# zhouzypaul/fql

Measured on AMD Instinct MI355X. Metric: FQL gradient-steps/s (batch=256), higher is better.
Workload: dtype f32

## Files before the change

### experiments/ab_inproc.py

```python
import os
import statistics
import sys
import time

sys.path.insert(0, os.path.dirname(os.path.dirname(os.path.abspath(__file__))))
import fql_amd
from tests.util import make_problem

envs = [dict(kv.split('=', 1) for kv in a.split()) if a.strip() and a.strip() != '-' else {} for a in sys.argv[1:3]]
rounds = int(sys.argv[3]) if len(sys.argv) > 3 else 7
n = int(sys.argv[4]) if len(sys.argv) > 4 else 300
prec = sys.argv[5] if len(sys.argv) > 5 else 'fp32'
B = int(sys.argv[6]) if len(sys.argv) > 6 else 256
H = 512
cfg, ds, batch, noise = make_problem(29, 8, B, (H,) * 4, seed=3)
cfg['precision'] = prec
agents = []
from fql_amd import _cabi
for e in envs:
    lib = e.pop('LIB', None)
    if lib:
        _cabi.LIB_PATH = os.path.abspath(lib)
        _cabi._lib = None
    e_show = dict(e, **({'LIB': lib} if lib else {}))
# ... 2 lines not shown
    a = fql_amd.FQLAgent.create(0, batch['observations'][:1], batch['actions'][:1], cfg)
    a.upload_dataset(ds)
    for _ in range(30):
        a.update_from_dataset(B)
    a.synchronize()
    agents.append(a)
    for k in e:
        del os.environ[k]
    e.update(e_show)
res = [[], []]
for r in range(rounds):
    for i, a in enumerate(agents):
        for _ in range(10):
            a.update_from_dataset(B)
        a.synchronize()
        t0 = time.perf_counter()
        for _ in range(n):
            a.update_from_dataset(B)
        a.synchronize()
        res[i].append((time.perf_counter() - t0) / n * 1e6)
for i, e in enumerate(envs):
    print(f'{"AB"[i]} {e}: median {statistics.median(res[i]):.1f} us/update  (min {min(res[i]):.1f}, max {max(res[i]):.1f})  = {1e6 / statistics.median(res[i]):.0f} updates/s')
print(f'B / A time: {statistics.median(res[1]) / statistics.median(res[0]):.4f}')
```

### fql_amd/csrc/fql_engine.hip

```cpp
#include "../../include/fql_amd.h"
#include "fql_kernels.h"
#include "fql_conv.h"
#include "fql_chain.h"
#include "fql_aux.h"
#include "fql_ifql.h"
#include "fql_rebrac.h"
#include "fql_sac.h"
#include "fql_bc.h"
#include "fql_iql.h"
#include "fql_iqld.h"
#include "fql_cfgrl.h"
#include <hip/hip_ext.h>
#include "fql_aql.h"

#include <algorithm>
#include <cmath>
#include <cstdarg>
#include <cstdio>
#include <cstdlib>
#include <cstring>
#include <map>
#include <memory>
#include <random>
#include <string>
// ... 138 lines not shown
    PrepArgs prep;
    PostOsArgs postos;
    LossCriticArgs lc;
    LossQArgs lq;
    LossBcArgs lb;
    LossActorArgs la;
    EulerFinishArgs ef;
    ConvArgs conv;
    PoolArgs pool;
    PoolBwdArgs poolb;
    ConvWgradArgs cw;
    ConvWredArgs cwr;
    EncDzArgs edz;
    ChainArgs chain;
    const ConvWprepTask* wprep_tasks = nullptr;
    int wprep_n = 0;
    int cw_grid = 0;
    int adam_c0 = 0, adam_n = -1;
    int adam_c1 = 0, adam_n1 = 0;
    int adam_polyak = -1;
    float adam_lr = 0.f;
    DevState* adam_st = nullptr;
    int fin_mode = 0;
    Bound k;
    int level = 0;
    int lane = 0;
    std::vector<int> deps;
};

struct Launch {
    OpType type;
    int grid = 0, ntasks = 0;
    size_t lds = 0;
    void* table = nullptr;
    Op op;
    bool pool_fused = false;
    int lane = 0;
    bool tmt2 = false, kbig = false, euler = false;
    double macs = 0.0;
    void *table_w = nullptr, *table_l = nullptr, *table_m = nullptr;
    int n_w = 0, n_l = 0, tile_w = 0, tile_l = 0, tile_m = 0;
    std::vector<GemmTask> dg_tasks;
    std::vector<GemmTask> h_gemm;
    std::vector<WgradTask> h_wgrad;
    std::vector<LnBwdTask> h_ln;
    std::vector<int> waits;
// ... 249 lines not shown
    float* in_noise[5] = {nullptr, nullptr, nullptr, nullptr, nullptr};
    int64_t* in_idx = nullptr;
    float *X_os = nullptr, *X_bc = nullptr, *X_eu = nullptr, *X_c1 = nullptr, *X_c2 = nullptr, *X_ct = nullptr;
    float *vel = nullptr, *w_rew = nullptr, *w_mask = nullptr, *w_act = nullptr, *tgt = nullptr;
    float *X_e0 = nullptr, *C0 = nullptr, *Abuf[2] = {nullptr, nullptr}, *Vpart = nullptr;
    bool fused_euler = false;
    bool use_chain = false;
    int fill_lane_full = 1;
    std::vector<float*> wf_bc;
    float *wf_w0 = nullptr, *wf_w4 = nullptr;
    WfragTask* d_wfrag = nullptr;
    int wfrag_n = 0, wfrag_grid = 0;
    std::vector<void*> chain_allocs;
    bool split_build = false;
    bool wide_tiles = false;
    bool split_ok = false;
    int vp_tiles = 0;
    int num_cus = 0;
    PassBuf p_os, p_os_bwd, p_bc, p_eu, p_c1[2], p_c2[2], p_ct[2];
    Program prog_fwdbwd, prog_opt, prog_loss;
    Program prog_opt_split;
    Program prog_full;
    int mod_chunk0[3] = {0, 0, 0}, mod_chunkn[3] = {0, 0, 0};
    Program prog_split;
    hipGraphExec_t split_exec[4] = {nullptr, nullptr, nullptr, nullptr};
    hipGraph_t split_graph[4] = {nullptr, nullptr, nullptr, nullptr};
    hipEvent_t ev_a = nullptr, ev_b = nullptr, ev_c = nullptr;
    bool split_begun = false;
    bool began = false;
    AqlRuntime aql;
    std::vector<AqlDispatch>* aql_rec = nullptr;
    bool last_update_aql = false;
    bool hip_dirty = true;
    void aql_drain() {
        if (!aql.up) return;
        try { aql.drain(); } catch (const AqlError& e) { throw HipError{e.msg}; }
    }

    float *ds_obs = nullptr, *ds_act = nullptr, *ds_rew = nullptr, *ds_mask = nullptr, *ds_nobs = nullptr;
    float* ds_row = nullptr;
    int64_t ds_size = 0, ds_cap = 0, ds_ptr = 0;
    unsigned char *ds_frames = nullptr, *ds_next_frames = nullptr;
    int64_t* ds_init = nullptr;
    int ds_fs = 0;
    float ds_paug = 0.f;
    float *rb_obs = nullptr, *rb_act = nullptr, *rb_rew = nullptr, *rb_mask = nullptr, *rb_nobs = nullptr;
// ... 397 lines not shown
        std::vector<int> range(n_train_leaves + 1, 0);
        for (const AdamChunk& c : ch) range[c.leaf + 1]++;
        for (int i = 0; i < n_train_leaves; ++i) range[i + 1] += range[i];
        {
            static const char* const trained[kNumKinds][3] = {
                {"modules_actor_bc_flow/", "modules_actor_onestep_flow/", "modules_critic/"},
                {"modules_actor_flow/", "modules_value/", "modules_critic/"},
                {"modules_actor/", "modules_critic/", "modules_critic/"},
                {"modules_actor/", "modules_alpha/", "modules_critic/"},
                {nullptr, nullptr, nullptr},
                {"modules_actor/", "modules_value/", "modules_critic/"},
                {"actor/", "value/", "critic/"},
                {nullptr, nullptr, nullptr}};
            const char* const* mods = trained[(int)kind];
            for (int m = 0; m < 3; ++m) {
                if (!mods[m]) { mod_chunk0[m] = 0; mod_chunkn[m] = n_chunks; continue; }
                int lo = 1 << 30, hi = -1;
                for (const Leaf& lf : leaves)
                    if (lf.trainable && lf.name.rfind(mods[m], 0) == 0) { lo = std::min(lo, lf.train_id); hi = std::max(hi, lf.train_id); }
                mod_chunk0[m] = range[lo];
                mod_chunkn[m] = range[hi + 1] - range[lo];
            }
        }
        HIP_CHECK(hipMalloc((void**)&d_leaf_range, range.size() * sizeof(int)));
        HIP_CHECK(hipMemcpy(d_leaf_range, range.data(), range.size() * sizeof(int), hipMemcpyHostToDevice));
        HIP_CHECK(hipMalloc((void**)&d_partials, (size_t)n_chunks * 4 * sizeof(float)));
        HIP_CHECK(hipMemset(d_partials, 0, (size_t)n_chunks * 4 * sizeof(float)));
    }

    const Leaf* find_leaf(const char* name) const {
        for (const Leaf& l : leaves)
            if (l.name == name) return &l;
        return nullptr;
    }
    static size_t leaf_count(const Leaf& l) {
        size_t n = 1;
        for (int i = 0; i < l.ndim; ++i) n *= (size_t)l.shape[i];
        return n;
    }
    void leaf_io(const Leaf& lf, float* arena, float* host, bool to_device) {
        HIP_CHECK(hipStreamSynchronize(stream));
        size_t ho = 0;
        for (const Segment& s : lf.segs) {
            HIP_CHECK(hipMemcpy2D(to_device ? (void*)(arena + s.off) : (void*)(host + ho), (to_device ? s.cols_p : s.cols) * sizeof(float),
                                  to_device ? (const void*)(host + ho) : (const void*)(arena + s.off),
                                  (to_device ? s.cols : s.cols_p) * sizeof(float), s.cols * sizeof(float), s.rows,
                                  to_device ? hipMemcpyHostToDevice : hipMemcpyDeviceToHost));
            ho += (size_t)s.rows * s.cols;
        }
    }
// ... 1168 lines not shown
                }
                else {
#define FQL_CHAIN_F32(HH, VV) FQL_LAUNCH((fql_chain_kernel<HH, VV>), dim3((L.op.chain.M / 16) * (HH / 32)), dim3(FQL_CHAIN_THREADS), FQL_CHAIN_LDS_BYTES(HH), s, ca)
                    if (cfg.actor_hidden[0] == 512) { if (ca.variant == 0) FQL_CHAIN_F32(512, 0); else if (ca.variant == 1) FQL_CHAIN_F32(512, 1); else if (ca.variant == 2) FQL_CHAIN_F32(512, 2); else FQL_CHAIN_F32(512, 3); }
                    else { if (ca.variant == 0) FQL_CHAIN_F32(256, 0); else if (ca.variant == 1) FQL_CHAIN_F32(256, 1); else if (ca.variant == 2) FQL_CHAIN_F32(256, 2); else FQL_CHAIN_F32(256, 3); }
#undef FQL_CHAIN_F32
                }
                break;
            }
            case OP_WFRAG:
                FQL_LAUNCH(fql_wfrag_kernel, dim3(wfrag_grid), dim3(FQL_THREADS), 0, s, (const WfragTask*)d_wfrag, wfrag_n, tl);
                break;
            case OP_DGRAD0: {
                Dgrad0Args a{};
                a.ntasks = (int)L.dg_tasks.size(); a.col0 = L.op.gemm.i1;
                for (int i = 0; i < a.ntasks; ++i) a.t[i] = L.dg_tasks[i];
                FQL_LAUNCH(fql_dgrad0_kernel, dim3(a.ntasks * (L.op.gemm.M / 16)), dim3(FQL_THREADS), 0, s, a);
                break;
            }
            case OP_HEAD_DGRAD:
                FQL_LAUNCH(fql_head_dgrad_kernel, dim3((L.op.gemm.M / 16) * (L.op.gemm.N / 64)), dim3(FQL_THREADS), 0, s, L.op.gemm);
                break;
            case OP_ADAM: {
                AdamArgs a{P, G, Mu, Nu, P + n_train, d_chunks, L.op.adam_st ? L.op.adam_st : d_state, d_partials, L.op.adam_c0,
                           L.op.adam_polyak >= 0 ? L.op.adam_polyak : (int)critic_size, L.op.adam_lr > 0.f ? L.op.adam_lr : cfg.lr, cfg.tau, tl,
                           L.op.adam_n1 > 0 ? L.op.adam_n : -1, L.op.adam_c1};
                FQL_LAUNCH(fql_adam_kernel, dim3(L.op.adam_n < 0 ? n_chunks : L.op.adam_n + L.op.adam_n1), dim3(FQL_THREADS), 0, s, a);
                break;
            }
            case OP_FINALIZE:
                FQL_LAUNCH(fql_finalize_kernel, dim3(1), dim3(FQL_THREADS), 0, s,
                                   FinalizeArgs{d_state, d_chunks, d_partials, d_leaf_range, n_chunks, n_train_leaves, L.op.fin_mode, tl});
                break;
            case OP_WGRAD: case OP_LNBWD: case OP_POSTOS: case OP_LOSS_CRITIC: case OP_LOSS_Q: case OP_LOSS_BC:
            case OP_PEC: case OP_XCHAIN: case OP_NUM_TYPES:
                throw HipError{"internal: op type " + std::to_string((int)L.type) + " has no launch of its own"};
            default: {
                const Bound& k = L.op.k;
                if (!k.fn) throw HipError{"internal: op type " + std::to_string((int)L.type) + " carries no bound launch"};
                alignas(16) unsigned char a[FQL_BOUND_BYTES];
                std::memcpy(a, k.args, (size_t)k.len);
                if (k.tl_at >= 0) std::memcpy(a + k.tl_at, &tl, sizeof tl);
                if (L.type == OP_IQLD_CFG) std::memcpy(a + offsetof(IqldCfgStepArgs, cfg), &sample_cfg, sizeof sample_cfg);
                void* argv[2] = {a + k.at[0], a + k.at[1]};
                if (aql_rec) aql_rec->push_back(AqlDispatch{k.fn, {k.grid, 1, 1}, {FQL_THREADS, 1, 1}, 0, std::vector<uint8_t>(a, a + k.len)});
                else if (prof_a) (void)hipExtLaunchKernel(k.fn, dim3(k.grid), dim3(FQL_THREADS), argv, 0, s, prof_a, prof_b, 0);
                else (void)hipLaunchKernel(k.fn, dim3(k.grid), dim3(FQL_THREADS), argv, 0, s);
                break;
            }
        }
    }

#undef FQL_LAUNCH
// ... 353 lines not shown
                if (t.K == 16 && t.N % 64 == 0 && t.M % 16 == 0 && (t.flags & GF_TRANS_B) && (t.flags & GF_GELUGRAD) && !(t.flags & (GF_BIAS | GF_RELUGRAD | GF_A_LN)) &&
                    cfg.precision != 1)
                    d.type = OP_HEAD_DGRAD;
                t.f0 = cfg.alpha * 2.0f / (float)(B * ad);
                d.reads.erase(std::remove(d.reads.begin(), d.reads.end(), (const void*)da), d.reads.end());
                for (const void* r : {(const void*)p_os.out, (const void*)tgt, (const void*)p_c2[0].dx0, (const void*)p_c2[1].dx0}) d.reads.push_back(r);
                d.writes.push_back(da);
                if (euler_finish_fused) {
                    const Net& nb = nets[NET_BC];
                    t.flags |= GF_A_EULFIN;
                    t.aux = Abuf[(fs - 1) & 1]; t.aux2 = Vpart; t.eb = P + nb.layers[nb.nl() - 1].b; t.f1 = 1.0f / (float)fs; t.ln_width = vp_tiles;
                    d.reads.erase(std::remove(d.reads.begin(), d.reads.end(), (const void*)tgt), d.reads.end());
                    for (const void* r : {(const void*)Abuf[(fs - 1) & 1], (const void*)Vpart, (const void*)(P + nb.layers[nb.nl() - 1].w)}) d.reads.push_back(r);
                    d.writes.push_back(tgt);
                }
            }
            if (euler_finish_fused) {
                const int keep = emit_lane;
                emit_lane = la_lane;
                push(pr, la_op);
                emit_lane = keep;
            }
            for (Op& w : os_w) {
                w.reads.push_back(p_os_bwd.dz[0]);
                emit_lane = 0;
                push(pr, w);
            }
            emit_lane = 0;
        }
        if (with_grads && visual) {
            place("enc", split_build ? 0 : 1, true);
            emit_encoder_backward(pr, eb_os, 0, B, p_os_bwd.dx0, nullptr, nets[NET_OS].in_p());
            if (enc_align) {
                emit_encoder_backward(pr, eb_c, 0, B, p_c1[0].dx0, p_c1[1].dx0, nets[NET_C0].in_p(), p_os_bwd.dx0);
                emit_encoder_backward(pr, eb_bc, 0, B, p_bc.dx0, nullptr, nets[NET_BC].in_p(), p_os_bwd.dx0);
            }
        }
        if (!with_grads) {
            Op op{};
            op.type = OP_FINALIZE;
            op.fin_mode = 0;
            op.reads = {I_CR, I_BC, I_Q, I_MSE, I_ACT};
            op.writes = {INFO};
            push(pr, op);
        }
    }

    void adam_for(Program& pr, int m, std::initializer_list<int> net_ids, int lane, int m2 = -1) {
        DevState* st = d_state;
            Op a{};
            a.type = OP_ADAM;
            a.adam_c0 = mod_chunk0[m]; a.adam_n = mod_chunkn[m];
            a.reads = {st};
            a.writes = {d_partials + mod_chunk0[m] * 4};
            if (m2 >= 0) { a.adam_c1 = mod_chunk0[m2]; a.adam_n1 = mod_chunkn[m2]; a.writes.push_back(d_partials + mod_chunk0[m2] * 4); }
            if (m2 == -2) {
                a.adam_c0 = 0; a.adam_n = -1;
                for (int mm = 0; mm < 3; ++mm) a.writes.push_back(d_partials + mod_chunk0[mm] * 4);
            }
            if (m == 2 && tgt) a.reads.push_back(tgt);
            for (int mm : {m, m2}) if (visual && mm >= 0) {
                const int m = mm;
                const int ei = m == 2 ? ENC_C : (m == 0 ? ENC_BC : ENC_OS);
                for (const EncStack& st : encs[ei].stacks)
                    for (const ConvL& c : st.conv) {
                        a.reads.push_back(G + c.w); a.reads.push_back(G + c.b);
                        a.writes.push_back(P + c.w);
                        if (m == 2) a.writes.push_back(P + n_train + c.w);
                    }
                const Layer& D = encs[ei].dense;
                a.reads.push_back(G + D.w); a.reads.push_back(G + D.b);
                a.writes.push_back(P + D.w);
                if (m == 2) a.writes.push_back(P + n_train + D.w);
            }
            for (int ni : net_ids)
                for (const Layer& L : nets[ni].layers) {
                    a.reads.push_back(G + L.w); a.reads.push_back(G + L.b);
                    a.writes.push_back(P + L.w);
                    if (L.ln) { a.reads.push_back(G + L.g); a.reads.push_back(G + L.be); a.writes.push_back(P + L.g); }
                    if (ni == NET_C0 || ni == NET_C1) a.writes.push_back(P + n_train + L.w);
                }
            emit_lane = lane;
            push(pr, a);
// ... 9 lines not shown
        } else {
            adam_for(pr, 2, {NET_C0, NET_C1, NET_BC, NET_OS}, 0, -2);
            if (use_chain) { emit_lane = 0; emit_wfrag(pr); }
        }
        Op f{};
        f.type = OP_FINALIZE;
        f.fin_mode = 1;
        f.reads = {d_partials + mod_chunk0[0] * 4, d_partials + mod_chunk0[1] * 4, d_partials + mod_chunk0[2] * 4, &st->info[0],
                   &st->info[4], &st->info[5], &st->info[7], &st->info[9]};
        f.writes = {&st->info[10], st};
        emit_lane = 0;
        push(pr, f);
    }
    void run_opt_split(hipStream_t s0, hipStream_t s1) {
        if (!ev_c) HIP_CHECK(hipEventCreateWithFlags(&ev_c, hipEventDisableTiming));
        if (!split_begun) HIP_CHECK(hipEventRecord(ev_c, s0));
        HIP_CHECK(hipStreamWaitEvent(s1, ev_c, 0));
        split_begun = false;
        const hipStream_t ls[FQL_LANES] = {s0, s1, s1, s1};
        run_launches(prog_opt_split, s0, ls, false);
    }

    void build_full_program(Program& pr) {
        build_step_program(pr, true);
        DevState* st = d_state;
        adam_for(pr, 2, {NET_C0, NET_C1, NET_BC}, fill_lane_full, 0);
        emit_wfrag(pr);
        adam_for(pr, 1, {NET_OS}, 0);
        Op f{};
        f.type = OP_FINALIZE;
        f.fin_mode = 1;
        f.reads = {d_partials + mod_chunk0[0] * 4, d_partials + mod_chunk0[1] * 4, d_partials + mod_chunk0[2] * 4, &st->info[0],
                   &st->info[4], &st->info[5], &st->info[7], &st->info[9]};
        f.writes = {&st->info[10], st};
        emit_lane = 0;
        push(pr, f);
    }

    FinalizeArgs fin_args(int do_grad_stats) const {
        return FinalizeArgs{d_state, d_chunks, d_partials, d_leaf_range, n_chunks, n_train_leaves, do_grad_stats, -1};
    }

    void build_ifql_program(Program& pr, bool with_grads) {
        const int od = cfg.obs_dim, ad = cfg.act_dim, ap = pad16(ad);
        DevState* st = d_state;
        const void *I_V = &st->info[IFQL_I_VALUE], *I_C = &st->info[IFQL_I_CRITIC], *I_A = &st->info[IFQL_I_ACTOR];
        wide_tiles = true;
        allow64 = true;
        emit_lane = 0;
        {
            Op op{};
            op.type = OP_IFQL_PREP;
            const IfqlPrepArgs iprep{d_src, st, seed, B, od, ad, nets[NET_OS].in_p(), nets[NET_C0].in_p(), nets[NET_BC].in_p(), ap,
                                     X_v, X_c1, X_bc, vel, w_rew, w_mask};
            op.k = bind(fql_ifql_prep_kernel, (iprep.B + 3) / 4, iprep);
            op.writes = {X_v, X_c1, X_bc, vel, w_rew, w_mask};
            push(pr, op);
        }
        emit_lane = 1;
// ... 1915 lines not shown
            std::vector<float> tab((size_t)(S + 1) * BC_EMB);
            for (int k = 0; k <= S; ++k) {
                const float t = (float)k / (float)S;
                const float ts = t * 10000.0f;
                for (int i = 0; i < BC_EMB / 2; ++i) {
                    const float freq = (float)std::exp(-std::log(10000.0) * (double)i / (double)(BC_EMB / 2));
                    const float arg = ts * freq;
                    tab[(size_t)k * BC_EMB + i] = (float)std::cos((double)arg);
                    tab[(size_t)k * BC_EMB + BC_EMB / 2 + i] = (float)std::sin((double)arg);
                }
            }
            HIP_CHECK(hipMalloc((void**)&h->d_emb, tab.size() * sizeof(float)));
            HIP_CHECK(hipMemcpy(h->d_emb, tab.data(), tab.size() * sizeof(float), hipMemcpyHostToDevice));
        }
        HIP_CHECK(hipMalloc((void**)&h->P, h->n_total * sizeof(float)));
        HIP_CHECK(hipMalloc((void**)&h->G, h->n_train * sizeof(float)));
        HIP_CHECK(hipMalloc((void**)&h->Mu, h->n_train * sizeof(float)));
        HIP_CHECK(hipMalloc((void**)&h->Nu, h->n_train * sizeof(float)));
        HIP_CHECK(hipMemset(h->G, 0, h->n_train * sizeof(float)));
        HIP_CHECK(hipMemset(h->Mu, 0, h->n_train * sizeof(float)));
        HIP_CHECK(hipMemset(h->Nu, 0, h->n_train * sizeof(float)));
        h->build_enc_weights();
        h->build_leaves();
        h->init_params();
        h->build_chain_weights();
        h->refresh_chain_weights(h->stream);
        HIP_CHECK(hipMalloc((void**)&h->d_state, sizeof(DevState)));
        if (h->own_info()) {
            HIP_CHECK(hipMalloc((void**)&h->iql_info, 2 * IQL_INFO_STRIDE * sizeof(float)));
            HIP_CHECK(hipMemset(h->iql_info, 0, 2 * IQL_INFO_STRIDE * sizeof(float)));
        }
        HIP_CHECK(hipMalloc((void**)&h->d_src, sizeof(SrcDesc)));
        HIP_CHECK(hipHostMalloc((void**)&h->h_src_ring, 64 * sizeof(SrcDesc), hipHostMallocDefault));
        HIP_CHECK(hipHostMalloc((void**)&h->h_info_ring, fql_engine::kInfoRing * 32 * sizeof(float), hipHostMallocDefault));
        for (auto& e : h->info_ev) HIP_CHECK(hipEventCreateWithFlags(&e, hipEventDisableTiming));
        DevState st{};
        st.rng_step = 0; st.adam_count = 0; st.train_step = 1; st.b1pow = 1.0; st.b2pow = 1.0; st.grad_scale = 1.0f; st.lam = 1.0f;
        const float ninf = -INFINITY, pinf = INFINITY;
        int bi; std::memcpy(&bi, &ninf, 4); st.gmax = bi >= 0 ? bi : bi ^ 0x7FFFFFFF;
        std::memcpy(&bi, &pinf, 4); st.gmin = bi >= 0 ? bi : bi ^ 0x7FFFFFFF;
        HIP_CHECK(hipMemcpy(h->d_state, &st, sizeof st, hipMemcpyHostToDevice));
        if (kind == AgentKind::IQLD) {
            HIP_CHECK(hipMalloc((void**)&h->d_state_a, sizeof(DevState)));
            HIP_CHECK(hipMemcpy(h->d_state_a, &st, sizeof st, hipMemcpyHostToDevice));
        }
        if (kind == AgentKind::CFGRL) {
// ... 2 lines not shown
            HIP_CHECK(hipHostMalloc((void**)&h->h_gsrc_ring, 64 * sizeof(CfgrlSrc), hipHostMallocDefault));
        }
        h->build_workspace(cfg->batch_size);
    } catch (const Invalid& e) {
        g_create_error = e.msg; fql_destroy(h); return FQL_E_INVALID;
    } catch (const HipError& e) {
        g_create_error = e.msg; fql_destroy(h); return FQL_E_HIP;
    }
    *out = h;
    return FQL_OK;
}

int fql_destroy(fql_handle h) {
    if (!h) return FQL_OK;
    if (h->group) { h->err = "fql_destroy: the handle is a member of an agent group (fql_group_destroy first)"; return FQL_E_STATE; }
    try { h->aql_drain(); } catch (...) {}
    if (h->stream) hipStreamSynchronize(h->stream);
    hipDeviceSynchronize();
    h->free_workspace();
    h->aql.shutdown();
    for (auto& kv : h->evals) {
        for (void* p : kv.second->allocs) hipFree(p);
    }
    hipFree(h->P); hipFree(h->G); hipFree(h->Mu); hipFree(h->Nu); hipFree(h->d_chunks); hipFree(h->d_partials); hipFree(h->d_leaf_range); hipFree(h->d_state); hipFree(h->d_src); hipFree(h->d_emb); hipFree(h->iql_info); hipFree(h->d_state_a);
    if (h->h_src_ring) hipHostFree(h->h_src_ring);
    hipFree(h->d_gsrc); hipFree(h->ds_final); hipFree(h->ds_reps);
    if (h->h_gsrc_ring) hipHostFree(h->h_gsrc_ring);
    if (h->h_info_ring) hipHostFree(h->h_info_ring);
    for (auto& e : h->info_ev) if (e) hipEventDestroy(e);
    hipFree(h->ds_obs); hipFree(h->ds_act); hipFree(h->ds_rew); hipFree(h->ds_mask); hipFree(h->ds_nobs); hipFree(h->ds_row);
    hipFree(h->ds_frames); hipFree(h->ds_next_frames); hipFree(h->ds_init);
    hipFree(h->rb_obs); hipFree(h->rb_act); hipFree(h->rb_rew); hipFree(h->rb_mask); hipFree(h->rb_nobs);
    hipFree(h->rb_frames); hipFree(h->rb_next_frames); hipFree(h->rb_init);
    for (void* q : h->enc_allocs) hipFree(q);
    for (void* q : h->chain_allocs) hipFree(q);
    if (h->stream) hipStreamDestroy(h->stream);
    for (hipStream_t s : h->lane_streams) if (s) hipStreamDestroy(s);
    delete h;
    return FQL_OK;
}

int fql_set_batch_size(fql_handle h, int batch_size) {
    if (!h) return FQL_E_INVALID;
    if (h->group) { h->err = "fql_set_batch_size: the handle is a member of an agent group (fql_group_destroy first)"; return FQL_E_STATE; }
    FQL_TRY(h, { if (batch_size != h->B) h->build_workspace(batch_size); });
}

// ... 1505 lines not shown
```

### fql_amd/csrc/fql_kernels.h

```cpp
#pragma once
#include <hip/hip_runtime.h>
#include <stdint.h>

typedef float f32x4 __attribute__((ext_vector_type(4)));

#define FQL_GAS __attribute__((address_space(1)))
__device__ __forceinline__ float ldg(const float* p) { return *(const FQL_GAS float*)p; }
__device__ __forceinline__ f32x4 ldg4(const float* p) { return *(const FQL_GAS f32x4*)p; }
__device__ __forceinline__ void stg(float* p, float v) { *(FQL_GAS float*)p = v; }
__device__ __forceinline__ void stg4(float* p, f32x4 v) { *(FQL_GAS f32x4*)p = v; }

#define FQL_THREADS 256

struct FastDiv {
    unsigned m;
    int d;
    __device__ __forceinline__ explicit FastDiv(int dd) : m(dd > 1 ? 0xFFFFFFFFu / (unsigned)dd + 1u : 0u), d(dd) {}
    __device__ __forceinline__ FastDiv(int dd, unsigned long long max_x) : m(dd > 1 && max_x * (unsigned long long)dd < (1ull << 32) ? 0xFFFFFFFFu / (unsigned)dd + 1u : 0u), d(dd) {}
    __device__ __forceinline__ int div(int x) const { return m ? (int)__umulhi((unsigned)x, m) : (d == 1 ? x : (int)((unsigned)x / (unsigned)d)); }
    __device__ __forceinline__ void divmod(int x, int& q, int& r) const { q = div(x); r = x - q * d; }
};

__device__ __forceinline__ float frcp(int d) { return __builtin_amdgcn_rcpf((float)d); }
__device__ __forceinline__ int sdiv(int x, float rd) { return (int)(((float)x + 0.5f) * rd); }
// ... 96 lines not shown
    int M, N, K;
    int lda, ldb, ldc;
    int ln_width;
    int flags;
    int tile0;
    int ntn;
    int wk;
    int tmt;
    int i0, i1, i2;
    float f0, f1;
    const float* ea_in;
    float* ea_out;
    const float* ew;
    const float* ew4;
    float* evp;
    const float* eb;
    int e_ntp;
    int xg;
#ifdef FQL_STAMPS
    unsigned long long* stamps64;
#endif
};

struct WgradTask {
    const float* X;
    const float* dZ;
    float* dW;
    float* db;
    int M, Kin, N;
    int ldx, ldz, ldw;
    int tile0, ntn;
};

struct LnBwdTask {
    const float* dY;
    const float* Z;
    const float* Gv;
    const float* stats;
    const float* gamma;
    float* dZ;
    float* dgamma;
    float* dbeta;
    int M, H, ld, width;
    int tile0, ntiles_rows;
    const float* dq;
    const float* wq;
    int ldq, ldw;
};

__device__ __forceinline__ float fast_tanh(float u) {
    const float e = __expf(-2.0f * fabsf(u));
    const float t = (1.0f - e) * __frcp_rn(1.0f + e);
    return copysignf(t, u);
}
// ... 1189 lines not shown
    }
    if (BIG && T.tmt == 2) {
        if (T.flags & GF_TRANS_B) gemm64_body<true, 2>(T, lds);
        else gemm64_body<false, 2>(T, lds);
    } else if (T.wk == 2) {
        if (T.flags & GF_TRANS_B) gemm32_body<true, 2>(T, lds);
        else gemm32_body<false, 2>(T, lds);
    } else {
        if (T.flags & GF_TRANS_B) gemm32_body<true, 1>(T, lds);
        else gemm32_body<false, 1>(T, lds);
    }
}

#define FQL_WGRAD_KT 32
#define FQL_WGRAD_LDS_FLOATS (4 * 8 * 64 * 4 + 4 * 64)
__device__ __forceinline__ void wgrad_load_chunk(f32x2 (&a)[8], f32x4 (&b)[8], const float* xp, const float* zp, unsigned xo, unsigned zo, size_t sx, size_t sz, int cnt) {
#pragma unroll
    for (int i = 0; i < 8; ++i) {
        const bool v = i < cnt;
        a[i] = v ? *(const FQL_GAS f32x2*)(xp + i * sx + xo) : f32x2{0.f, 0.f};
        b[i] = v ? ldg4(zp + i * sz + zo) : f32x4{0.f, 0.f, 0.f, 0.f};
    }
}
template <int NU>
__device__ __forceinline__ void wgrad_finish(const WgradTask& T, float* lds, const f32x4 (&acc)[NU][4], const float (&bs)[4], int tk, int k0, int n0,
                                             int ntv, bool xv) {
    float* red = lds;
    float (*redb)[64] = reinterpret_cast<float (*)[64]>(lds + 4 * 4 * NU * 64 * 4);
    const int wave = threadIdx.x >> 6, lane = threadIdx.x & 63;
    const int c = lane & 15, q = lane >> 4;
#pragma unroll
    for (int t = 0; t < 4; ++t) {
#pragma unroll
        for (int u = 0; u < NU; ++u) *reinterpret_cast<f32x4*>(&red[((wave * 4 * NU + 4 * u + t) * 64 + lane) * 4]) = acc[u][t];
        float v = bs[t];
        v += __shfl_xor(v, 16);
        v += __shfl_xor(v, 32);
        if (q == 0) redb[wave][4 * c + t] = v;
    }
    __syncthreads();
    if (xv && 4 * q + wave < 4 * ntv) {
#pragma unroll
        for (int u = 0; u < NU; ++u) {
            f32x4 r;
#pragma unroll
            for (int t = 0; t < 4; ++t) {
                float v = red[((0 * 4 * NU + 4 * u + t) * 64 + lane) * 4 + wave];
#pragma unroll
                for (int w = 1; w < 4; ++w) v += red[((w * 4 * NU + 4 * u + t) * 64 + lane) * 4 + wave];
                r[t] = v;
            }
            stg4(T.dW + (size_t)(k0 + NU * c + u) * T.ldw + n0 + 16 * q + 4 * wave, r);
        }
    }
    if (tk == 0 && T.db && wave == 0 && lane < 16 * ntv) T.db[n0 + lane] = redb[0][lane] + redb[1][lane] + redb[2][lane] + redb[3][lane];
}
__device__ __forceinline__ void wgrad_body(const WgradTask& T, int bid, float* lds) {
    const int local = bid - T.tile0;
    const int tk = sdiv(local, frcp(T.ntn)), tn = local - tk * T.ntn;
    const int wave = __builtin_amdgcn_readfirstlane(threadIdx.x >> 6), lane = threadIdx.x & 63;
    const int c = lane & 15, q = lane >> 4;
    const int k0 = tk * FQL_WGRAD_KT, n0 = tn * 64;
    const int ntv = min(4, (T.N - n0) >> 4);
    const bool xv = k0 + 2 * c < T.Kin;
    const int steps = T.M >> 4;
    const size_t sx = (size_t)4 * T.ldx, sz = (size_t)4 * T.ldz;
    const float* __restrict__ xp = T.X + (size_t)(4 * wave * steps) * T.ldx;
    const float* __restrict__ zp = T.dZ + (size_t)(4 * wave * steps) * T.ldz;
    const unsigned xo = (unsigned)(q * T.ldx + min(k0 + 2 * c, T.Kin - 2)), zo = (unsigned)(q * T.ldz + n0 + min(4 * c, 16 * ntv - 4));
    f32x4 acc[2][4];
#pragma unroll
    for (int t = 0; t < 4; ++t) acc[0][t] = acc[1][t] = f32x4{0.f, 0.f, 0.f, 0.f};
    float bs[4] = {0.f, 0.f, 0.f, 0.f};
    f32x2 a0[8], a1[8];
    f32x4 b0[8], b1[8];
    auto mma = [&](const f32x2(&a)[8], const f32x4(&b)[8]) {
#pragma unroll
        for (int i = 0; i < 8; ++i)
#pragma unroll
            for (int t = 0; t < 4; ++t) {
                bs[t] += b[i][t];
                acc[0][t] = __builtin_amdgcn_mfma_f32_16x16x4f32(b[i][t], a[i][0], acc[0][t], 0, 0, 0);
                acc[1][t] = __builtin_amdgcn_mfma_f32_16x16x4f32(b[i][t], a[i][1], acc[1][t], 0, 0, 0);
            }
    };
    wgrad_load_chunk(a0, b0, xp, zp, xo, zo, sx, sz, steps);
    for (int s = 0; s < steps; s += 16) {
        if (s + 8 < steps) wgrad_load_chunk(a1, b1, xp + (s + 8) * sx, zp + (s + 8) * sz, xo, zo, sx, sz, steps - s - 8);
        mma(a0, b0);
        if (s + 8 < steps) {
            if (s + 16 < steps) wgrad_load_chunk(a0, b0, xp + (s + 16) * sx, zp + (s + 16) * sz, xo, zo, sx, sz, steps - s - 16);
            mma(a1, b1);
        }
    }
    wgrad_finish<2>(T, lds, acc, bs, tk, k0, n0, ntv, xv);
}
#define FQL_WGRAD_KT_SPLIT 16
__device__ __forceinline__ void wgrad_split_body(const WgradTask& T, int bid, float* lds) {
    const int local = bid - T.tile0;
    const int tk = sdiv(local, frcp(T.ntn)), tn = local - tk * T.ntn;
    const int wave = __builtin_amdgcn_readfirstlane(threadIdx.x >> 6), lane = threadIdx.x & 63;
    const int c = lane & 15, q = lane >> 4;
    const int k0 = tk * FQL_WGRAD_KT_SPLIT, n0 = tn * 64;
    const int ntv = min(4, (T.N - n0) >> 4);
    const bool zv = c < 4 * ntv;
    const int steps = T.M >> 4;
    const size_t sx = (size_t)4 * T.ldx, sz = (size_t)4 * T.ldz;
    const float* __restrict__ xp = T.X + (size_t)(4 * wave * steps) * T.ldx;
    const float* __restrict__ zp = T.dZ + (size_t)(4 * wave * steps) * T.ldz;
    const unsigned xo = (unsigned)(q * T.ldx + k0 + c), zo = (unsigned)(q * T.ldz + n0 + min(4 * c, 16 * ntv - 4));
    f32x4 acc[1][4];
#pragma unroll
    for (int t = 0; t < 4; ++t) acc[0][t] = f32x4{0.f, 0.f, 0.f, 0.f};
    float bs[4] = {0.f, 0.f, 0.f, 0.f};
    float a0[8], a1[8];
    f32x4 b0[8], b1[8];
    auto load = [&](float (&a)[8], f32x4 (&b)[8], int s0) {
#pragma unroll
// ... 17 lines not shown
            for (int i = 0; i < 4; ++i) {
                unsigned h, l;
                const float b0v = (s0 + 2 * i < steps && zv) ? b[2 * i][t] : 0.f;
                const float b1v = (s0 + 2 * i + 1 < steps && zv) ? b[2 * i + 1][t] : 0.f;
                bs[t] += b0v + b1v;
                bsplit2(b0v, b1v, h, l);
                bh[i] = h; bl[i] = l;
            }
            acc[0][t] = mfma_bf16(bh, al, acc[0][t]);
            acc[0][t] = mfma_bf16(bl, ah, acc[0][t]);
            acc[0][t] = mfma_bf16(bh, ah, acc[0][t]);
            __builtin_amdgcn_sched_barrier(0);
        }
    };
    load(a0, b0, 0);
    for (int s = 0; s < steps; s += 16) {
        if (s + 8 < steps) load(a1, b1, s + 8);
        mma(a0, b0, s);
        if (s + 8 < steps) {
            if (s + 16 < steps) load(a0, b0, s + 16);
            mma(a1, b1, s + 8);
        }
    }
    wgrad_finish<1>(T, lds, acc, bs, tk, k0, n0, ntv, true);
}

template <bool SYN>
__device__ __forceinline__ void lnbwd_body(const LnBwdTask& T, int bid, float (*red)[16][16]) {
    const int local = bid - T.tile0;
    const int wave = threadIdx.x >> 6, lane = threadIdx.x & 63;
    if (local < T.ntiles_rows) {
        const int row = local * 4 + wave;
        if (row >= T.M) return;
        const float mean = ldg(T.stats + 2 * row), rstd = ldg(T.stats + 2 * row + 1);
        const float* dy = T.dY + (size_t)row * T.ld;
        const float* z = T.Z + (size_t)row * T.ld;
        const float* gv = T.Gv + (size_t)row * T.ld;
        const float dqr = SYN ? ldg(T.dq + (size_t)row * T.ldq) : 0.f;
        f32x4 zz[4], dd[4], gm[4], gq[4];
#pragma unroll
        for (int i = 0; i < 4; ++i) {
            const int k4 = 4 * (lane + 64 * i);
            if (k4 < T.H) {
                zz[i] = ldg4(z + k4);
                gq[i] = ldg4(gv + k4);
                gm[i] = ldg4(T.gamma + k4);
                if (SYN) {
// ... 47 lines not shown
                    dv[u] = SYN ? ldg(T.dq + (size_t)m * T.ldq) * wc : ldg(T.dY + (size_t)m * T.ld + col);
                    zv[u] = ldg(T.Gv + (size_t)m * T.ld + col);
                }
#pragma unroll
                for (int u = 0; u < 16; ++u) {
                    if (m0 + 16 * u < T.M) {
                        const float xh = (zv[u] - st[u][0]) * st[u][1];
                        sg += dv[u] * xh; sb += dv[u];
                    }
                }
            }
        }
        red[0][rg][cc] = sg; red[1][rg][cc] = sb;
        __syncthreads();
        if (rg == 0 && col < T.H) {
            float g = 0.f, b = 0.f;
#pragma unroll
            for (int r = 0; r < 16; ++r) { g += red[0][r][cc]; b += red[1][r][cc]; }
            stg(T.dgamma + col, (col < T.width) ? g : 0.f);
            stg(T.dbeta + col, (col < T.width) ? b : 0.f);
        }
    }
}

struct DevState {
    uint64_t rng_step;
    uint64_t rng_stream;
    int64_t adam_count;
    int64_t train_step;
    double b1pow, b2pow;
    float grad_scale;
    float lam;
    float info[16];
    float gmax_bits_pad;
    int gmax, gmin;
    float leaf_sumsq[256];
};

struct SrcDesc {
    const float *obs, *act, *rew, *mask, *nobs;
    const int64_t* idx;
    const float *eps1, *x0, *t, *z, *eps2;
    int64_t lo, span;
    int use_rng_idx;
    int advance;
    int split;
    const float *obs2, *act2, *rew2, *mask2, *nobs2;
    int64_t lo2, span2;
    const float* nact;
    int64_t nact_rows;
};

struct PrepArgs {
    const SrcDesc* src;
    DevState* st;
    uint64_t key;
    int B, od, ad;
    int inp_c, inp_b;
    int ap;
    float *X_os, *X_bc, *X_eu, *X_c1, *X_c2, *X_ct, *vel, *w_rew, *w_mask, *w_act;
// ... 242 lines not shown

enum : int { MISC_POSTOS = 0, MISC_LOSS_CRITIC, MISC_LOSS_Q, MISC_LOSS_BC };
struct MiscTask {
    int kind;
    union {
        PostOsArgs po;
        LossCriticArgs lc;
        LossQArgs lq;
        LossBcArgs lb;
    };
};

struct AdamChunk { int off, len, leaf; };
struct AdamArgs {
    float *P, *G, *Mu, *Nu, *T;
    const AdamChunk* chunks;
    DevState* st;
    float* partials;
    int chunk0;
    int critic_size;
    float lr, tau;
    int tl;
    int n0, chunk1;
};
__device__ __forceinline__ int f2ord(float f) {
    const int i = __float_as_int(f);
    return i >= 0 ? i : i ^ 0x7FFFFFFF;
}
__device__ __forceinline__ float ord2f(int i) { return __int_as_float(i >= 0 ? i : i ^ 0x7FFFFFFF); }

__device__ __forceinline__ void fql_adam_body(const AdamArgs& A) {
    __shared__ float sh[4];
    tl_enter(A.tl);
    const int cidx = (A.n0 < 0 || (int)blockIdx.x < A.n0) ? (int)blockIdx.x + A.chunk0 : (int)blockIdx.x - A.n0 + A.chunk1;
    const AdamChunk ch = A.chunks[cidx];
    const float c1 = (float)(1.0 - A.st->b1pow * 0.9), c2 = (float)(1.0 - A.st->b2pow * 0.999);
    const float gsc = A.st->grad_scale;
    float ss = 0.f, mx = -INFINITY, mn = INFINITY;
    const int n4 = ch.len >> 2;
#pragma unroll
    for (int it = 0; it < 4; ++it) {
        const int i = threadIdx.x + it * FQL_THREADS;
        if (i < n4) {
            const int o = ch.off + 4 * i;
            f32x4 g = ldg4(A.G + o);
            const f32x4 p = ldg4(A.P + o);
            f32x4 m = ldg4(A.Mu + o);
            f32x4 v = ldg4(A.Nu + o);
            f32x4 pn;
#pragma unroll
            for (int e = 0; e < 4; ++e) {
                const float ge = g[e] * gsc;
                m[e] = 0.9f * m[e] + 0.1f * ge;
                v[e] = 0.999f * v[e] + 0.001f * ge * ge;
                const float mh = m[e] / c1, vh = v[e] / c2;
                pn[e] = p[e] - A.lr * (mh / (sqrtf(vh) + 1e-8f));
                ss += ge * ge; mx = fmaxf(mx, ge); mn = fminf(mn, ge);
            }
            stg4(A.Mu + o, m);
            stg4(A.Nu + o, v);
            stg4(A.P + o, pn);
            if (o < A.critic_size) {
                f32x4 t = ldg4(A.T + o);
#pragma unroll
                for (int e = 0; e < 4; ++e) t[e] = p[e] * A.tau + t[e] * (1.0f - A.tau);
                stg4(A.T + o, t);
            }
        }
    }
    const float tss = block_sum(ss, sh);
    const float tmx = block_max(mx, sh), tmn = -block_max(-mn, sh);
    if (threadIdx.x == 0) {
        float* pp = A.partials + 4 * (size_t)cidx;
        pp[0] = tss; pp[1] = tmx; pp[2] = tmn;
    }
    tl_exit(A.tl);
}
__global__ __launch_bounds__(FQL_THREADS) void fql_adam_kernel(AdamArgs A) { fql_adam_body(A); }
__global__ __launch_bounds__(FQL_THREADS) void fql_adam_multi_kernel(const AdamArgs* __restrict__ args) { const AdamArgs A = ((const FQL_CONST_AS AdamArgs*)args)[blockIdx.y]; fql_adam_body(A); }

struct FinalizeArgs {
    DevState* st;
    const AdamChunk* chunks;
    const float* partials;
    const int* leaf_range;
    int n_chunks, nleaves, do_grad_stats;
    int tl;
};
__device__ __forceinline__ void fql_finalize_body(const FinalizeArgs& A) {
    __shared__ float sh[4];
    __shared__ float leafn[256];
    DevState* st = A.st;
    tl_enter(A.tl);
    if (!A.do_grad_stats) return;
    float mx = -INFINITY, mn = INFINITY;
    for (int cidx = threadIdx.x; cidx < A.n_chunks; cidx += FQL_THREADS) {
// ... 161 lines not shown
```

Measured before the change: 2875.

## Fuse one-step actor Adam update into its weight-gradient kernel epilogue

Adds an optional path, on by default and disabled with FQL_FUSE_OS_ADAM=0, where the one-step flow actor's weight-gradient kernels apply the Adam update directly in their finish stage. Each kernel writes per-tile gradient statistics into a new partials layout that the finalize kernel consumes. This removes the separate Adam launch for the one-step net and a re-read of its gradients. In exchange it adds register and memory traffic to the wgrad epilogue, uses a different partials slot mapping, and only applies to non-visual, non-layer-norm FQL runs without split precision.

```diff
diff --git a/experiments/ab_inproc.py b/experiments/ab_inproc.py
--- a/experiments/ab_inproc.py
+++ b/experiments/ab_inproc.py
@@ -48,3 +48,5 @@
 for i, e in enumerate(envs):
     print(f'{"AB"[i]} {e}: median {statistics.median(res[i]):.1f} us/update  (min {min(res[i]):.1f}, max {max(res[i]):.1f})  = {1e6 / statistics.median(res[i]):.0f} updates/s')
 print(f'B / A time: {statistics.median(res[1]) / statistics.median(res[0]):.4f}')
+pairs = [b / a for a, b in zip(*res)]
+print('B / A per round: ' + ' '.join(f'{p:.4f}' for p in pairs) + f'   mean {statistics.mean(pairs):.4f}  min {min(pairs):.4f}  max {max(pairs):.4f}')
diff --git a/fql_amd/csrc/fql_engine.hip b/fql_amd/csrc/fql_engine.hip
--- a/fql_amd/csrc/fql_engine.hip
+++ b/fql_amd/csrc/fql_engine.hip
@@ -184,6 +184,7 @@
     float adam_lr = 0.f;
     DevState* adam_st = nullptr;
     int fin_mode = 0;
+    bool fused_tail = false;
     Bound k;
     int level = 0;
     int lane = 0;
@@ -479,6 +480,13 @@
     Program prog_opt_split;
     Program prog_full;
     int mod_chunk0[3] = {0, 0, 0}, mod_chunkn[3] = {0, 0, 0};
+    bool fuse_os_env = true;
+    bool fuse_os_adam = false;
+    std::vector<int> h_leaf_range;
+    float* d_partials_f = nullptr;
+    int* d_leaf_range_f = nullptr;
+    int n_slots_f = 0, os_pshift = 0;
+    std::vector<int> os_slot_w, os_slot_b;
     Program prog_split;
     hipGraphExec_t split_exec[4] = {nullptr, nullptr, nullptr, nullptr};
     hipGraph_t split_graph[4] = {nullptr, nullptr, nullptr, nullptr};
@@ -922,10 +930,47 @@
                 mod_chunkn[m] = range[hi + 1] - range[lo];
             }
         }
+        h_leaf_range = range;
         HIP_CHECK(hipMalloc((void**)&d_leaf_range, range.size() * sizeof(int)));
         HIP_CHECK(hipMemcpy(d_leaf_range, range.data(), range.size() * sizeof(int), hipMemcpyHostToDevice));
         HIP_CHECK(hipMalloc((void**)&d_partials, (size_t)n_chunks * 4 * sizeof(float)));
         HIP_CHECK(hipMemset(d_partials, 0, (size_t)n_chunks * 4 * sizeof(float)));
+    }
+
+    int wgrad_ntn(int N) const { return (N + 63) / 64; }
+    int wgrad_ntk(int Kin) const {
+        const int wkt = cfg.precision == 2 ? FQL_WGRAD_KT_SPLIT : FQL_WGRAD_KT;
+        return (Kin + wkt - 1) / wkt;
+    }
+    void build_fused_slots() {
+        if (kind != AgentKind::FQL || visual || cfg.actor_layer_norm) return;
+        const Net& n = nets[NET_OS];
+        const int os_lo = mod_chunk0[1], os_hi = mod_chunk0[1] + mod_chunkn[1];
+        std::vector<int> range(n_train_leaves + 1, 0);
+        os_slot_w.assign(n.nl(), -1); os_slot_b.assign(n.nl(), -1);
+        for (const Leaf& lf : leaves) {
+            if (!lf.trainable) continue;
+            const int t = lf.train_id;
+            int cnt = h_leaf_range[t + 1] - h_leaf_range[t];
+            if (h_leaf_range[t] >= os_lo && h_leaf_range[t] < os_hi) {
+                if (lf.segs.size() != 1 || lf.segs[0].chunk_w > 0) return;
+                cnt = -1;
+                for (int l = 0; l < n.nl(); ++l) {
+                    const Layer& ly = n.layers[l];
+                    if (lf.segs[0].off == ly.w) { os_slot_w[l] = range[t]; cnt = wgrad_ntk(ly.in_p) * wgrad_ntn(ly.out_p); }
+                    else if (lf.segs[0].off == ly.b) { os_slot_b[l] = range[t]; cnt = wgrad_ntn(ly.out_p); }
+                }
+                if (cnt < 0) return;
+            }
+            range[t + 1] = range[t] + cnt;
+        }
+        for (int l = 0; l < n.nl(); ++l) if (os_slot_w[l] < 0 || os_slot_b[l] < 0) return;
+        n_slots_f = range[n_train_leaves];
+        os_pshift = n_slots_f - n_chunks;
+        HIP_CHECK(hipMalloc((void**)&d_leaf_range_f, range.size() * sizeof(int)));
+        HIP_CHECK(hipMemcpy(d_leaf_range_f, range.data(), range.size() * sizeof(int), hipMemcpyHostToDevice));
+        HIP_CHECK(hipMalloc((void**)&d_partials_f, (size_t)n_slots_f * 4 * sizeof(float)));
+        HIP_CHECK(hipMemset(d_partials_f, 0, (size_t)n_slots_f * 4 * sizeof(float)));
     }
 
     const Leaf* find_leaf(const char* name) const {
@@ -2140,13 +2185,18 @@
                 FQL_LAUNCH(fql_head_dgrad_kernel, dim3((L.op.gemm.M / 16) * (L.op.gemm.N / 64)), dim3(FQL_THREADS), 0, s, L.op.gemm);
                 break;
             case OP_ADAM: {
-                AdamArgs a{P, G, Mu, Nu, P + n_train, d_chunks, L.op.adam_st ? L.op.adam_st : d_state, d_partials, L.op.adam_c0,
+                const bool ft = L.op.fused_tail;
+                AdamArgs a{P, G, Mu, Nu, P + n_train, d_chunks, L.op.adam_st ? L.op.adam_st : d_state, ft ? d_partials_f : d_partials, L.op.adam_c0,
                            L.op.adam_polyak >= 0 ? L.op.adam_polyak : (int)critic_size, L.op.adam_lr > 0.f ? L.op.adam_lr : cfg.lr, cfg.tau, tl,
-                           L.op.adam_n1 > 0 ? L.op.adam_n : -1, L.op.adam_c1};
+                           L.op.adam_n1 > 0 ? L.op.adam_n : -1, L.op.adam_c1, mod_chunk0[1] + mod_chunkn[1], ft ? os_pshift : 0};
                 FQL_LAUNCH(fql_adam_kernel, dim3(L.op.adam_n < 0 ? n_chunks : L.op.adam_n + L.op.adam_n1), dim3(FQL_THREADS), 0, s, a);
                 break;
             }
             case OP_FINALIZE:
+                if (L.op.fused_tail)
+                    FQL_LAUNCH(fql_finalize_kernel, dim3(1), dim3(FQL_THREADS), 0, s,
+                                       FinalizeArgs{d_state, d_chunks, d_partials_f, d_leaf_range_f, n_slots_f, n_train_leaves, L.op.fin_mode, tl});
+                else
                 FQL_LAUNCH(fql_finalize_kernel, dim3(1), dim3(FQL_THREADS), 0, s,
                                    FinalizeArgs{d_state, d_chunks, d_partials, d_leaf_range, n_chunks, n_train_leaves, L.op.fin_mode, tl});
                 break;
@@ -2546,6 +2596,22 @@
                 emit_lane = keep;
             }
             for (Op& w : os_w) {
+                if (fuse_os_adam) {
+                    const Net& n = nets[NET_OS];
+                    int l = 0;
+                    while (l < n.nl() && w.wgrad.dW != G + n.layers[l].w) ++l;
+                    if (l >= n.nl()) invalid("internal: a one-step weight gradient matches no layer");
+                    const Layer& ly = n.layers[l];
+                    WgradAdam& a = w.wgrad.ad;
+                    a.P = P + ly.w; a.Mu = Mu + ly.w; a.Nu = Nu + ly.w;
+                    a.Pb = P + ly.b; a.Mub = Mu + ly.b; a.Nub = Nu + ly.b;
+                    a.st = st; a.lr = cfg.lr;
+                    a.part = d_partials_f + 4 * (size_t)os_slot_w[l]; a.partb = d_partials_f + 4 * (size_t)os_slot_b[l];
+                    w.reads.push_back(st);
+                    for (const void* p : {(const void*)a.P, (const void*)a.Pb, (const void*)a.Mu, (const void*)a.Mub, (const void*)a.Nu, (const void*)a.Nub,
+                                          (const void*)a.part, (const void*)a.partb})
+                        w.writes.push_back(p);
+                }
                 w.reads.push_back(p_os_bwd.dz[0]);
                 emit_lane = 0;
                 push(pr, w);
@@ -2583,6 +2649,7 @@
                 for (int mm = 0; mm < 3; ++mm) a.writes.push_back(d_partials + mod_chunk0[mm] * 4);
             }
             if (m == 2 && tgt) a.reads.push_back(tgt);
+            a.fused_tail = fuse_os_adam;
             for (int mm : {m, m2}) if (visual && mm >= 0) {
                 const int m = mm;
                 const int ei = m == 2 ? ENC_C : (m == 0 ? ENC_BC : ENC_OS);
@@ -2638,19 +2705,24 @@
     }
 
     void build_full_program(Program& pr) {
+        fuse_os_adam = fuse_os_env && d_partials_f && !visual && !cfg.actor_layer_norm && cfg.precision != 2;
         build_step_program(pr, true);
         DevState* st = d_state;
         adam_for(pr, 2, {NET_C0, NET_C1, NET_BC}, fill_lane_full, 0);
         emit_wfrag(pr);
-        adam_for(pr, 1, {NET_OS}, 0);
+        if (!fuse_os_adam) adam_for(pr, 1, {NET_OS}, 0);
         Op f{};
         f.type = OP_FINALIZE;
         f.fin_mode = 1;
+        f.fused_tail = fuse_os_adam;
         f.reads = {d_partials + mod_chunk0[0] * 4, d_partials + mod_chunk0[1] * 4, d_partials + mod_chunk0[2] * 4, &st->info[0],
                    &st->info[4], &st->info[5], &st->info[7], &st->info[9]};
+        if (fuse_os_adam)
+            for (size_t l = 0; l < os_slot_w.size(); ++l) { f.reads.push_back(d_partials_f + 4 * (size_t)os_slot_w[l]); f.reads.push_back(d_partials_f + 4 * (size_t)os_slot_b[l]); }
         f.writes = {&st->info[10], st};
         emit_lane = 0;
         push(pr, f);
+        fuse_os_adam = false;
     }
 
     FinalizeArgs fin_args(int do_grad_stats) const {
@@ -4612,6 +4684,11 @@
         HIP_CHECK(hipMemset(h->Nu, 0, h->n_train * sizeof(float)));
         h->build_enc_weights();
         h->build_leaves();
+        {
+            const char* e = getenv("FQL_FUSE_OS_ADAM");
+            h->fuse_os_env = !(e && atoi(e) == 0);
+        }
+        h->build_fused_slots();
         h->init_params();
         h->build_chain_weights();
         h->refresh_chain_weights(h->stream);
@@ -4660,7 +4737,7 @@
     for (auto& kv : h->evals) {
         for (void* p : kv.second->allocs) hipFree(p);
     }
-    hipFree(h->P); hipFree(h->G); hipFree(h->Mu); hipFree(h->Nu); hipFree(h->d_chunks); hipFree(h->d_partials); hipFree(h->d_leaf_range); hipFree(h->d_state); hipFree(h->d_src); hipFree(h->d_emb); hipFree(h->iql_info); hipFree(h->d_state_a);
+    hipFree(h->P); hipFree(h->G); hipFree(h->Mu); hipFree(h->Nu); hipFree(h->d_chunks); hipFree(h->d_partials); hipFree(h->d_leaf_range); hipFree(h->d_partials_f); hipFree(h->d_leaf_range_f); hipFree(h->d_state); hipFree(h->d_src); hipFree(h->d_emb); hipFree(h->iql_info); hipFree(h->d_state_a);
     if (h->h_src_ring) hipHostFree(h->h_src_ring);
     hipFree(h->d_gsrc); hipFree(h->ds_final); hipFree(h->ds_reps);
     if (h->h_gsrc_ring) hipHostFree(h->h_gsrc_ring);
diff --git a/fql_amd/csrc/fql_kernels.h b/fql_amd/csrc/fql_kernels.h
--- a/fql_amd/csrc/fql_kernels.h
+++ b/fql_amd/csrc/fql_kernels.h
@@ -142,6 +142,28 @@
 #endif
 };
 
+struct DevState {
+    uint64_t rng_step;
+    uint64_t rng_stream;
+    int64_t adam_count;
+    int64_t train_step;
+    double b1pow, b2pow;
+    float grad_scale;
+    float lam;
+    float info[16];
+    float gmax_bits_pad;
+    int gmax, gmin;
+    float leaf_sumsq[256];
+};
+
+struct WgradAdam {
+    float *P, *Mu, *Nu;
+    float *Pb, *Mub, *Nub;
+    const DevState* st;
+    float* part;
+    float* partb;
+    float lr;
+};
 struct WgradTask {
     const float* X;
     const float* dZ;
@@ -150,6 +172,7 @@
     int M, Kin, N;
     int ldx, ldz, ldw;
     int tile0, ntn;
+    WgradAdam ad;
 };
 
 struct LnBwdTask {
@@ -1385,13 +1408,34 @@
         b[i] = v ? ldg4(zp + i * sz + zo) : f32x4{0.f, 0.f, 0.f, 0.f};
     }
 }
+__device__ __forceinline__ float adam_elem(float ge, float p, float& m, float& v, float lr, float c1, float c2) {
+    m = fmaf(ge, 0.1f, 0.9f * m);
+    v = fmaf(ge, 0.001f * ge, 0.999f * v);
+    const float mh = m / c1, vh = v / c2;
+    return fmaf(-lr, mh / (sqrtf(vh) + 1e-8f), p);
+}
 template <int NU>
-__device__ __forceinline__ void wgrad_finish(const WgradTask& T, float* lds, const f32x4 (&acc)[NU][4], const float (&bs)[4], int tk, int k0, int n0,
+__device__ __forceinline__ void wgrad_finish(const WgradTask& T, float* lds, const f32x4 (&acc)[NU][4], const float (&bs)[4], int local, int tk, int k0, int n0,
                                              int ntv, bool xv) {
     float* red = lds;
     float (*redb)[64] = reinterpret_cast<float (*)[64]>(lds + 4 * 4 * NU * 64 * 4);
     const int wave = threadIdx.x >> 6, lane = threadIdx.x & 63;
     const int c = lane & 15, q = lane >> 4;
+    const bool adam = T.ad.P != nullptr;
+    const bool own = xv && 4 * q + wave < 4 * ntv;
+    f32x4 pp[NU], pm[NU], pv[NU];
+    float c1 = 1.f, c2 = 1.f, gsc = 1.f;
+    if (adam) {
+        c1 = (float)(1.0 - T.ad.st->b1pow * 0.9); c2 = (float)(1.0 - T.ad.st->b2pow * 0.999);
+        gsc = T.ad.st->grad_scale;
+        if (own) {
+#pragma unroll
+            for (int u = 0; u < NU; ++u) {
+                const size_t o = (size_t)(k0 + NU * c + u) * T.ldw + n0 + 16 * q + 4 * wave;
+                pp[u] = ldg4(T.ad.P + o); pm[u] = ldg4(T.ad.Mu + o); pv[u] = ldg4(T.ad.Nu + o);
+            }
+        }
+    }
 #pragma unroll
     for (int t = 0; t < 4; ++t) {
 #pragma unroll
@@ -1402,7 +1446,8 @@
         if (q == 0) redb[wave][4 * c + t] = v;
     }
     __syncthreads();
-    if (xv && 4 * q + wave < 4 * ntv) {
+    float ss = 0.f, mx = -INFINITY, mn = INFINITY;
+    if (own) {
 #pragma unroll
         for (int u = 0; u < NU; ++u) {
             f32x4 r;
@@ -1413,10 +1458,61 @@
                 for (int w = 1; w < 4; ++w) v += red[((w * 4 * NU + 4 * u + t) * 64 + lane) * 4 + wave];
                 r[t] = v;
             }
-            stg4(T.dW + (size_t)(k0 + NU * c + u) * T.ldw + n0 + 16 * q + 4 * wave, r);
-        }
-    }
-    if (tk == 0 && T.db && wave == 0 && lane < 16 * ntv) T.db[n0 + lane] = redb[0][lane] + redb[1][lane] + redb[2][lane] + redb[3][lane];
+            const size_t o = (size_t)(k0 + NU * c + u) * T.ldw + n0 + 16 * q + 4 * wave;
+            stg4(T.dW + o, r);
+            if (adam) {
+                f32x4 pn;
+#pragma unroll
+                for (int e = 0; e < 4; ++e) {
+                    const float ge = r[e] * gsc;
+                    float me = pm[u][e], ve = pv[u][e];
+                    pn[e] = adam_elem(ge, pp[u][e], me, ve, T.ad.lr, c1, c2);
+                    pm[u][e] = me; pv[u][e] = ve;
+                    ss += ge * ge; mx = fmaxf(mx, ge); mn = fminf(mn, ge);
+                }
+                stg4(T.ad.Mu + o, pm[u]);
+                stg4(T.ad.Nu + o, pv[u]);
+                stg4(T.ad.P + o, pn);
+            }
+        }
+    }
+    if (tk == 0 && T.db && wave == 0) {
+        const bool bv = lane < 16 * ntv;
+        float b = 0.f;
+        if (bv) {
+            b = redb[0][lane] + redb[1][lane] + redb[2][lane] + redb[3][lane];
+            T.db[n0 + lane] = b;
+        }
+        if (adam) {
+            float bss = 0.f, bmx = -INFINITY, bmn = INFINITY;
+            if (bv) {
+                const float ge = b * gsc;
+                float m = T.ad.Mub[n0 + lane], v = T.ad.Nub[n0 + lane];
+                const float pn = adam_elem(ge, T.ad.Pb[n0 + lane], m, v, T.ad.lr, c1, c2);
+                T.ad.Mub[n0 + lane] = m; T.ad.Nub[n0 + lane] = v; T.ad.Pb[n0 + lane] = pn;
+                bss = ge * ge; bmx = ge; bmn = ge;
+            }
+#pragma unroll
+            for (int o = 1; o < 64; o <<= 1) { bss += __shfl_xor(bss, o); bmx = fmaxf(bmx, __shfl_xor(bmx, o)); bmn = fminf(bmn, __shfl_xor(bmn, o)); }
+            if (lane == 0) {
+                float* sl = T.ad.partb + 4 * (size_t)(n0 >> 6);
+                sl[0] = bss; sl[1] = bmx; sl[2] = bmn;
+            }
+        }
+    }
+    if (adam) {
+#pragma unroll
+        for (int o = 1; o < 64; o <<= 1) { ss += __shfl_xor(ss, o); mx = fmaxf(mx, __shfl_xor(mx, o)); mn = fminf(mn, __shfl_xor(mn, o)); }
+        __syncthreads();
+        if (lane == 0) { red[4 * wave] = ss; red[4 * wave + 1] = mx; red[4 * wave + 2] = mn; }
+        __syncthreads();
+        if (threadIdx.x == 0) {
+            float* sl = T.ad.part + 4 * (size_t)local;
+            sl[0] = red[0] + red[4] + red[8] + red[12];
+            sl[1] = fmaxf(fmaxf(red[1], red[5]), fmaxf(red[9], red[13]));
+            sl[2] = fminf(fminf(red[2], red[6]), fminf(red[10], red[14]));
+        }
+    }
 }
 __device__ __forceinline__ void wgrad_body(const WgradTask& T, int bid, float* lds) {
     const int local = bid - T.tile0;
@@ -1456,7 +1552,7 @@
             mma(a1, b1);
         }
     }
-    wgrad_finish<2>(T, lds, acc, bs, tk, k0, n0, ntv, xv);
+    wgrad_finish<2>(T, lds, acc, bs, local, tk, k0, n0, ntv, xv);
 }
 #define FQL_WGRAD_KT_SPLIT 16
 __device__ __forceinline__ void wgrad_split_body(const WgradTask& T, int bid, float* lds) {
@@ -1520,7 +1616,7 @@
             mma(a1, b1, s + 8);
         }
     }
-    wgrad_finish<1>(T, lds, acc, bs, tk, k0, n0, ntv, true);
+    wgrad_finish<1>(T, lds, acc, bs, local, tk, k0, n0, ntv, true);
 }
 
 template <bool SYN>
@@ -1614,20 +1710,6 @@
         }
     }
 }
-
-struct DevState {
-    uint64_t rng_step;
-    uint64_t rng_stream;
-    int64_t adam_count;
-    int64_t train_step;
-    double b1pow, b2pow;
-    float grad_scale;
-    float lam;
-    float info[16];
-    float gmax_bits_pad;
-    int gmax, gmin;
-    float leaf_sumsq[256];
-};
 
 struct SrcDesc {
     const float *obs, *act, *rew, *mask, *nobs;
@@ -1916,6 +1998,7 @@
     float lr, tau;
     int tl;
     int n0, chunk1;
+    int pshift_from, pshift;
 };
 __device__ __forceinline__ int f2ord(float f) {
     const int i = __float_as_int(f);
@@ -1945,10 +2028,9 @@
 #pragma unroll
             for (int e = 0; e < 4; ++e) {
                 const float ge = g[e] * gsc;
-                m[e] = 0.9f * m[e] + 0.1f * ge;
-                v[e] = 0.999f * v[e] + 0.001f * ge * ge;
-                const float mh = m[e] / c1, vh = v[e] / c2;
-                pn[e] = p[e] - A.lr * (mh / (sqrtf(vh) + 1e-8f));
+                float me = m[e], ve = v[e];
+                pn[e] = adam_elem(ge, p[e], me, ve, A.lr, c1, c2);
+                m[e] = me; v[e] = ve;
                 ss += ge * ge; mx = fmaxf(mx, ge); mn = fminf(mn, ge);
             }
             stg4(A.Mu + o, m);
@@ -1965,7 +2047,7 @@
     const float tss = block_sum(ss, sh);
     const float tmx = block_max(mx, sh), tmn = -block_max(-mn, sh);
     if (threadIdx.x == 0) {
-        float* pp = A.partials + 4 * (size_t)cidx;
+        float* pp = A.partials + 4 * (size_t)(cidx + (cidx >= A.pshift_from ? A.pshift : 0));
         pp[0] = tss; pp[1] = tmx; pp[2] = tmn;
     }
     tl_exit(A.tl);
```

After: 2871. No clear change (-0.2%).
